# netneurolab/pypyls

Hardware: AMD Instinct MI355X
Metric: resamples/sec (perm+boot), behavioral_pls X(500x200000)/Y(500x50) fp64 (higher is better)
Workload: dtype f64

## Files before the change

### pypyls_amd/csrc/plsx_core.hip

```cpp
#include "plsx_internal.h"
#include "plsx_resample.h"
using namespace plsxi;

namespace plsxi {

const char* const kKernelClassNames[KC_COUNT] = {"k_xprod", "k_gram", "k_small", "k_urot", "k_nt_gemm",
                                                 "k_ucorr_partial", "k_simpls_dual", "k_build_A", "k_xprod_moments",
                                                 "k_sd_cv_score", "k_sd_coef", "k_coef_prod", "k_percentile", "k_contrast", "k_mb_rownorm"};

int plan_groups(plsx_ctx* c)
{
    const bool mb = c->method == PLSX_MULTIBLOCK;
    c->scaled = ((c->method == PLSX_BEHAVIORAL || mb) && !c->cov) ? 1 : 0;
    c->momrows = ((c->method == PLSX_BEHAVIORAL && (!c->cov || c->cv_mom)) || (mb && !c->cov)) ? 1 : 0;
    const int Jw = c->momrows ? c->J : 0;
    c->gps = 0;
    c->h_slice_row0.clear(); c->h_slice_rows.clear(); c->h_slice_cell0.clear(); c->h_slice_ncell.clear();
    auto fit = [&](int mt) {
        int b = 0;
        for (int n = 1; n <= 512; ++n) {
            int td = ceil_div(n * c->Tp, 16), tw = Jw ? ceil_div(n * Jw, 16) : 0;
            if (td + 2 * tw <= mt && tw * 16 <= 48) b = n; else break;
        }
        return b;
// ... 202 lines not shown
        if (waste < 0.03) break;
    }
    return best;
}

SmallArgs small_args(plsx_ctx* ctx, int mode)
{
    SmallArgs a;
    memset(&a, 0, sizeof(a));
    a.mode = mode; a.n = ctx->Tp; a.L = ctx->L; a.rotate = 1;
    a.G = ptr<double>(ctx->Gm); a.P = ptr<double>(ctx->Pm);
    a.V0 = ptr<double>(ctx->V0); a.d0 = ptr<double>(ctx->d0);
    a.Mfrag = ptr<double>(ctx->Mfrag); a.nks_t = ctx->nks_t; a.LT = ctx->LT;
    a.status = ptr<int>(ctx->status);
    return a;
}

bool plsc_single_pass(const plsx_ctx* ctx)
{
    return ctx->method != PLSX_REGRESSION && !ctx->scaled && use_dual(ctx) && ctx->gps == 0 && ctx->L == ctx->Tp &&
           ctx->Tp <= PLSX_JACOBI_TP && 2 * (size_t)ctx->L * PLSX_ACC_PITCH * 8 <= 72 * 1024 && !ctx->opt[OPT_TWO_PASS_BOOT];
}

int note_spectrum(plsx_ctx* ctx, const double* d_sv, hipStream_t st)
{
    std::vector<double> d(ctx->L);
    HIPCHK(hipMemcpyAsync(d.data(), d_sv, (size_t)ctx->L * 8, hipMemcpyDeviceToHost, st));
    HIPCHK(hipStreamSynchronize(st));
    double dmax = 0.0;
    for (double v : d) if (v > dmax) dmax = v;
    int graded = 0;
    for (double v : d) if (v > PLSX_RANK_RTOL * dmax && v < PLSX_REFINE_TAU * dmax) graded = 1;
    if (graded != ctx->graded) ctx->has_Kd = ctx->has_Kd && !graded;
    ctx->graded = graded && !ctx->opt[OPT_NO_REFINE];
    return 0;
}

int run_contrast_norms(plsx_ctx* ctx, int nres, double* out_sv, hipStream_t st)
{
    const int ntiles = ceil_div(ctx->B, 16);
    const int tpc = std::max(32, round_up(ceil_div(ntiles, 64), 4));
    const int nchunk = ceil_div(ntiles, tpc);
    const int LTl = ceil_div(ctx->nc, 16);
    if (int e = ensure(ctx, ctx->cpart, (size_t)nres * nchunk * ctx->L * 8)) return e;
    KTimer tm(ctx, KC_CONTRAST, st);
    for (int lt0 = 0; lt0 < LTl; lt0 += 4) {
        const int ltc = std::min(4, LTl - lt0);
        const size_t lds = (size_t)ctx->nks_t * ltc * 512;
        const bool vlds = lds <= 64 * 1024;
#define CN_ARGS ptr<double>(ctx->R), ctx->strideR, ctx->Bpad, ctx->nks_t, ptr<double>(ctx->Cfrag), ctx->LT, lt0, ctx->B, \
                tpc, ctx->L, ptr<double>(ctx->cpart)
#define CN_CASE(N) case N: \
            if (vlds) { HIPCHK(set_lds((k_contrast_norms<N, true>), lds)); \
                        hipLaunchKernelGGL((k_contrast_norms<N, true>), dim3(nchunk, nres), dim3(256), lds, st, CN_ARGS); } \
            else hipLaunchKernelGGL((k_contrast_norms<N, false>), dim3(nchunk, nres), dim3(256), 0, st, CN_ARGS); \
// ... 44 lines not shown
    if (!c) return PLSX_ERR_HIP;
    c->device = device;
    if (hipMalloc(&c->status.p, 4 * sizeof(int)) != hipSuccess || hipMemset(c->status.p, 0, 4 * sizeof(int)) != hipSuccess) {
        delete c;
        return PLSX_ERR_HIP;
    }
    c->status.bytes = 4 * sizeof(int);
    *out = c;
    return PLSX_OK;
} PLSX_CATCH(nullptr)

int plsx_ctx_destroy(plsx_ctx* ctx)
try {
    if (!ctx) return PLSX_OK;
    (void)hipSetDevice(ctx->device);
    (void)hipDeviceSynchronize();
    (void)plsx_comm_destroy(ctx);
    for (Buf* b : {&ctx->Xc, &ctx->xmean, &ctx->Y, &ctx->cell_of_row, &ctx->cell_start, &ctx->cell_len,
                   &ctx->out_row, &ctx->mom_idx, &ctx->mom_n, &ctx->Afrag, &ctx->R, &ctx->Gm, &ctx->Pm,
                   &ctx->part, &ctx->Mfrag, &ctx->U0T, &ctx->V0, &ctx->d0, &ctx->tmpW,
                   &ctx->Rfull, &ctx->Vp, &ctx->dp, &ctx->Mvd, &ctx->Cm, &ctx->srcx, &ctx->srcy, &ctx->part2,
                   &ctx->Kmat, &ctx->swork, &ctx->spct, &ctx->sc,
                   &ctx->momout, &ctx->R2, &ctx->cvc, &ctx->Qm, &ctx->Vs, &ctx->ds, &ctx->ybar, &ctx->pred,
                   &ctx->Xn, &ctx->out_row_f, &ctx->mom_idx_f, &ctx->Kd, &ctx->Ad, &ctx->Wd, &ctx->gws, &ctx->cellS, &ctx->rowc, &ctx->out_row_s, &ctx->okx, &ctx->oky, &ctx->psum, &ctx->psq, &ctx->row_slice, &ctx->row_local, &ctx->slice_cell0, &ctx->cell_momrow, &ctx->status, &ctx->ScT, &ctx->out_row_w, &ctx->Qs, &ctx->out_row_d, &ctx->mom_idx_d, &ctx->Afrag_m, &ctx->momn_m, &ctx->scale,
                   &ctx->Afrag_c, &ctx->rank_c, &ctx->rowtab_c, &ctx->m1_c, &ctx->m2_c, &ctx->out_row_c, &ctx->mom_idx_c, &ctx->mask_c,
                   &ctx->refV, &ctx->refLam, &ctx->refK0, &ctx->refPart, &ctx->refPartP, &ctx->refH, &ctx->flipws, &ctx->pflags,
                   &ctx->Cq, &ctx->Vsumq, &ctx->Vdq, &ctx->Cc, &ctx->Asumc, &ctx->Adc, &ctx->Qc, &ctx->cichunk, &ctx->cpA, &ctx->cppart, &ctx->colsd, &ctx->Zcv, &ctx->cvpsrc, &ctx->cvpfit, &ctx->shrsum, &ctx->shq, &ctx->shG, &ctx->shKG, &ctx->Vtq, &ctx->Afrag_q, &ctx->qpart, &ctx->ccon, &ctx->sFt, &ctx->Yrot,
                   &ctx->Cv, &ctx->Cfrag, &ctx->cpart, &ctx->mbpart})
        release(*b);
    for (auto& ev : ctx->events) { (void)hipEventDestroy(ev.e0); (void)hipEventDestroy(ev.e1); }
    delete ctx;
    return PLSX_OK;
} PLSX_CATCH(ctx)

const char* plsx_last_error(const plsx_ctx* ctx) { return ctx ? ctx->err.c_str() : "null context"; }

int plsx_sync(plsx_ctx* ctx)
try {
    if (!ctx) return PLSX_ERR_ARG;
    HIPCHK(hipSetDevice(ctx->device));
    HIPCHK(hipDeviceSynchronize());
    int stw[4] = {0, 0, 0, 0};
    HIPCHK(hipMemcpy(stw, ctx->status.p, 4 * sizeof(int), hipMemcpyDeviceToHost));
    if (stw[1] || stw[2]) {
        ctx->n_refined += stw[1];
        ctx->n_unrefined += stw[2];
        HIPCHK(hipMemset(static_cast<int*>(ctx->status.p) + 1, 0, 2 * sizeof(int)));
// ... 312 lines not shown
try {
    NEED_DATA();
    if (!d_W || !d_out || L < 1) return fail(ctx, PLSX_ERR_ARG, "plsx_project: bad arguments");
    hipStream_t st = static_cast<hipStream_t>(stream);
    HIPCHK(hipSetDevice(ctx->device));
    if (int e = ensure(ctx, ctx->tmpW, (size_t)L * ctx->Bpad * 8)) return e;
    HIPCHK(hipMemsetAsync(ctx->tmpW.p, 0, (size_t)L * ctx->Bpad * 8, st));
    hipLaunchKernelGGL(k_transpose, dim3(ceil_div(L, 32), ceil_div(ctx->B, 32)), dim3(32, 8), 0, st,
                       d_W, ctx->B, L, L, ptr<double>(ctx->tmpW), ctx->Bpad);
    LAUNCHCHK();
    return run_nt(ctx, ptr<double>(ctx->Xc), 0, ctx->Bpad, ctx->S, ptr<double>(ctx->tmpW), 0, ctx->Bpad, L,
                  nullptr, 0, 0, 0, ctx->B, 1, d_out, 0, L, nullptr, 0, 0, st);
} PLSX_CATCH(ctx)

int plsx_set_original(plsx_ctx* ctx, const double* d_xw, const double* d_sv, const double* d_yw,
                      void* stream)
try {
    NEED_DATA();
    if (!d_xw || !d_sv || !d_yw) return fail(ctx, PLSX_ERR_ARG, "plsx_set_original: null input");
    hipStream_t st = static_cast<hipStream_t>(stream);
    HIPCHK(hipSetDevice(ctx->device));
    HIPCHK(hipMemcpyAsync(ctx->V0.p, d_yw, (size_t)ctx->Tp * ctx->L * 8, hipMemcpyDeviceToDevice, st));
    HIPCHK(hipMemcpyAsync(ctx->d0.p, d_sv, (size_t)ctx->L * 8, hipMemcpyDeviceToDevice, st));
    if (int e = note_spectrum(ctx, d_sv, st)) return e;
    hipLaunchKernelGGL(k_transpose, dim3(ceil_div(ctx->L, 32), ceil_div(ctx->B, 32)), dim3(32, 8), 0, st,
                       d_xw, ctx->B, ctx->L, ctx->L, ptr<double>(ctx->U0T), ctx->Bpad);
    LAUNCHCHK();
    if (int e = run_nt(ctx, ptr<double>(ctx->Xc), 0, ctx->Bpad, ctx->S, ptr<double>(ctx->U0T), 0, ctx->Bpad,
                       ctx->L, nullptr, 0, 0, 0, ctx->B, 1, ptr<double>(ctx->Xc) + ctx->B, 0, ctx->Bpad,
                       nullptr, 0, 0, st))
        return e;
    {
        const int Sd = round_up(ctx->S, 8);
        if (int e = ensure(ctx, ctx->ScT, (size_t)ctx->L * Sd * 8, true)) return e;
        HIPCHK(hipMemsetAsync(ctx->ScT.p, 0, (size_t)ctx->L * Sd * 8, st));
        hipLaunchKernelGGL(k_transpose, dim3(ceil_div(ctx->L, 32), ceil_div(ctx->S, 32)), dim3(32, 8), 0, st,
                           ptr<double>(ctx->Xc) + ctx->B, ctx->S, ctx->L, ctx->Bpad, ptr<double>(ctx->ScT), Sd);
        LAUNCHCHK();
    }
    ctx->has_orig = true; ctx->quad_active = 0;
    return PLSX_OK;
} PLSX_CATCH(ctx)

}

namespace plsxi {

// ... 61 lines not shown
                               ptr<int>(ctx->cell_of_row), idx, lay, ptr<double>(ctx->Ad), (size_t)0, Sd,
                               -1);
        }
        LAUNCHCHK();
        if (int e = run_nt(ctx, ptr<double>(ctx->Ad), 0, Sd, m * Tp, ptr<double>(ctx->Kd), 0, Sd, S,
                           nullptr, 0, 0, 0, S, 1, ptr<double>(ctx->Wd), 0, Sd, nullptr, 0, 0, st))
            return e;
        if (int e = run_dual_gp(ctx, m, Sd, nullptr, 0, st)) return e;
        if (ctx->nc > 0) {
            KTimer tm(ctx, KC_CONTRAST, st);
            hipLaunchKernelGGL(k_contrast_quad, dim3(m), dim3(256), 0, st, ptr<double>(ctx->Gm), Tp, ptr<double>(ctx->Cv),
                               ctx->L, ctx->nc, d_out_sv + (size_t)off * ctx->L);
            LAUNCHCHK();
            continue;
        }
        SmallArgs a = small_args(ctx, SMALL_PERM);
        a.rotate = rotate ? 1 : 0;
        a.out_sv = d_out_sv + (size_t)off * ctx->L;
        if (int e = run_small(ctx, a, m, st)) return e;
    }
    return PLSX_OK;
}

int perm_batch_impl(plsx_ctx* ctx, const int32_t* d_perm_idx, const double* d_ystack, int n, int rotate,
                    double* d_out_sv, void* stream)
{
    hipStream_t st = static_cast<hipStream_t>(stream);
    HIPCHK(hipSetDevice(ctx->device));
    if (use_dual(ctx)) return perm_dual(ctx, d_perm_idx, d_ystack, n, rotate, d_out_sv, st);
    const int pg = ctx->fix ? ctx->npgf : ctx->npg;
    const int nb = balanced_batch(n, launch_groups(ctx, n, pg) * pg, pg);
    for (int off = 0; off < n; off += nb) {
        const int m = std::min(nb, n - off);
        const int* idx = d_perm_idx ? d_perm_idx + (size_t)off * ctx->S : nullptr;
        const bool perm_y = ctx->method == PLSX_BEHAVIORAL || ctx->method == PLSX_MULTIBLOCK;
        const int* xs = perm_y ? nullptr : idx;
        const int* ys = perm_y ? idx : nullptr;
        const double* yst = d_ystack ? d_ystack + (size_t)off * ctx->S * ctx->T : nullptr;
        if (ctx->fix) {
            if (int e = run_xprod_fixed(ctx, ys, m, st, yst)) return e;
        } else if (int e = run_xprod(ctx, xs, ys, m, st, false, yst)) return e;
        if (ctx->nc > 0) {
            if (int e = run_contrast_norms(ctx, m, d_out_sv + (size_t)off * ctx->L, st)) return e;
            continue;
        }
        if (int e = run_gram(ctx, m, false, st)) return e;
        SmallArgs a = small_args(ctx, SMALL_PERM);
        a.rotate = rotate ? 1 : 0;
        a.out_sv = d_out_sv + (size_t)off * ctx->L;
        if (int e = run_small(ctx, a, m, st, ptr<double>(ctx->R))) return e;
    }
    return PLSX_OK;
}

}

namespace plsxi {

int quad_accumulate(plsx_ctx* ctx, int m, hipStream_t st, const QuadSet* qs)
{
    const int S = ctx->S, L = qs ? qs->L : (ctx->method == PLSX_REGRESSION ? ctx->ncomp : ctx->L);
// ... 394 lines not shown
try {
    plsx_ctx* ctx = const_cast<plsx_ctx*>(cctx);
    if (!ctx || !out || cap < 1) return PLSX_ERR_ARG;
    double ms = 0.0;
    int launches = 0;
    for (auto& ev : ctx->events) {
        if (ev.cls != KC_XPROD) continue;
        float t = 0.f;
        if (hipEventSynchronize(ev.e1) == hipSuccess && hipEventElapsedTime(&t, ev.e0, ev.e1) == hipSuccess)
            ms += t;
        ++launches;
    }
    double crows = 0.0;
    if (ctx->last_compact_n > 0) {
        std::vector<int> cnt(ctx->last_compact_n);
        if (hipMemcpy(cnt.data(), ptr<int>(ctx->rowtab_c) + (size_t)ctx->last_compact_n * ctx->last_compact_ktot,
                      cnt.size() * sizeof(int), hipMemcpyDeviceToHost) == hipSuccess) {
            for (int c : cnt) crows += 4.0 * ((std::max(c, 1) + 3) / 4);
            crows /= (double)cnt.size() * ctx->S;
        }
    }
    const bool cmp = ctx->last_compact_n > 0;
    const auto uvar = [&](int nks) { return (double)(nks > 0 && ctx->urot_tail_l ? nks + 100 : nks); };
    double vals[22] = {ms, (double)launches, (double)(cmp ? 1 : (ctx->sepmom_used ? ctx->npg_d : ctx->npg)),
                       (double)(cmp ? ceil_div(ctx->Tp, 16) : (ctx->sepmom_used ? ctx->MTd : ctx->MT)),
                       (double)ctx->Gcap * ctx->npg, (double)ctx->timed_units, (double)use_dual(ctx), crows,
                       ctx->nt_flops, (double)ctx->quad_series, (double)ctx->quad_MT, (double)ctx->quad_gpl,
                       (double)ctx->urot_waves_l, (double)ctx->urot_splits_l, (double)ctx->urot_rps_l,
                       uvar(ctx->urot_nks_first), (double)ctx->gram_chunks_l, uvar(ctx->urot_nks_last),
                       (double)ctx->gram_kind_l, (double)ctx->split_blocks_l, (double)ctx->split_reader_l,
                       (double)(cmp && ctx->last_moment_rows ? 1 : 0)};
    int n = std::min(cap, 22);
    for (int i = 0; i < n; ++i) out[i] = vals[i];
    return n;
} PLSX_CATCH(const_cast<plsx_ctx*>(cctx))

int plsx_kernel_timing(const plsx_ctx* cctx, int kernel_class, double* ms_out, int* launches_out)
try {
    plsx_ctx* ctx = const_cast<plsx_ctx*>(cctx);
    if (!ctx || kernel_class < 0 || kernel_class >= KC_COUNT) return PLSX_ERR_ARG;
    double ms = 0.0;
    int launches = 0;
    for (auto& ev : ctx->events) {
        if (ev.cls != kernel_class) continue;
        float t = 0.f;
        if (hipEventSynchronize(ev.e1) == hipSuccess && hipEventElapsedTime(&t, ev.e0, ev.e1) == hipSuccess)
            ms += t;
        ++launches;
    }
    if (ms_out) *ms_out = ms;
    if (launches_out) *launches_out = launches;
    return PLSX_OK;
} PLSX_CATCH(const_cast<plsx_ctx*>(cctx))

const char* plsx_kernel_class_name(int kernel_class)
// ... 146 lines not shown
```

### pypyls_amd/csrc/plsx_internal.h

```cpp
#pragma once
#include "plsx_kernels.h"
#include <chrono>
#include "../../include/plsx.h"

#include <algorithm>
#include <cmath>
#include <cstdio>
#include <cstdlib>
#include <cstring>
#include <new>
#include <stdexcept>
#include <string>
#include <thread>
#include <vector>

struct Buf {
    void* p = nullptr;
    size_t bytes = 0;
};

enum {
    OPT_NO_REFINE = 0, OPT_MIN_BATCH, OPT_INBLOCK_MOMENTS, OPT_NO_COMPACT_BOOT, OPT_COMPACT_BOOT_ALWAYS,
    OPT_SEPMOM_ALWAYS, OPT_NO_GRAM4, OPT_UROT_GENERIC, OPT_UROT_NO_TAIL4, OPT_NO_FIXED_X, OPT_NO_DUAL_PERM,
    OPT_TWO_PASS_BOOT, OPT_SPLIT_INBLOCK, OPT_NO_SPLIT_FUSE, OPT_SPLIT_TWO_READERS, OPT_EXPECT_RESAMPLES,
    OPT_SIMPLS_JACOBI, OPT_PERCENTILE_SORT, OPT_QUAD_SUMS, OPT_SPLIT_READER8, OPT_SIMPLS_GLOBAL,
    OPT_CROSSCOV_SPARSE, OPT_NO_MOMENT_ROWS, OPT_COUNT
};
static const char* const kOptionNames[OPT_COUNT] = {
    "no_refine", "min_batch", "inblock_moments", "no_compact_boot", "compact_boot_always",
    "sepmom_always", "no_gram4", "urot_generic", "urot_no_tail4", "no_fixed_x", "no_dual_perm",
    "two_pass_boot", "split_inblock", "no_split_fuse", "split_two_readers", "expect_resamples",
    "simpls_jacobi", "percentile_sort", "quad_sums", "split_reader8", "simpls_global",
    "crosscov_sparse", "no_moment_rows"};

#ifndef PLSX_CKT
#define PLSX_CKT 3
#endif

struct plsx_ctx {
    int device = 0;
    std::string err;
    int opt[OPT_COUNT] = {};
    bool has_data = false, has_orig = false;
    int method = 0, S = 0, B = 0, T = 0, J = 0, n_groups = 0, n_cond = 1, mc = 0, cov = 0;
    int Tp = 0, Tpp = 0, L = 0, Kpad = 0, nks = 0, Bx = 0, Bpad = 0;
    int MT = 24, npg = 0, w0 = 0, sq0 = 0, nmom_pad = 0, scaled = 0, momrows = 0, Gcap = 0, Galloc = 0;
    int nks_t = 0, LT = 0, cv_mom = 0;
    int afrag_group0 = 0;
    int sepmom = 0, MTd = 0, npg_d = 0, sepmom_used = 0;
    size_t group_stride_d = 0;
    Buf out_row_d, mom_idx_d, Afrag_m, momn_m, scale;
    Buf Afrag_c, rank_c, rowtab_c, m1_c, m2_c, out_row_c, mom_idx_c, mask_c;
    int has_compact_maps = 0;
    size_t group_stride = 0;
    int gps = 0;
    Buf row_slice, row_local, slice_cell0, cell_momrow;
// ... 11 lines not shown
    Buf Kd, Ad, Wd;
    Buf Zcv;
    Buf cvpsrc, cvpfit;
    Buf shrsum, shq, shG, shKG;
    int has_shrsum = 0;
    Buf Qs;
    Buf ScT, out_row_w;
    int npg_w = 0;
    Buf gws;
    Buf status;
    Buf pflags;
    Buf flipws;
    Buf refV, refLam, refK0, refPart, refPartP, refH, Yrot;
    int graded = 0;
    long long n_refined = 0, n_unrefined = 0;
    Buf cellS, rowc, out_row_s;
    Buf ccon, sFt;
    int split_blocks_l = 0, split_reader_l = 0;
    int has_sFt = 0, split_raw = 0;
    int has_cellS = 0;
    int nc = 0;
    Buf Cv, Cfrag, cpart;
    Buf mbpart;
    int dual = 0, dual_ok = 0, has_Kd = 0;
    Buf okx, oky;
    Buf psum, psq;
    Buf Cq, Vsumq, Vdq, Vtq, Afrag_q, qpart;
    int quad_active = 0;
    long long quad_n = 0, series_total = 0;
    Buf Cc, Asumc, Adc, Qc;
    int coef_active = 0, coef_c = 0;
    long long coef_n = 0;
    double* keepA = nullptr;
    long long keep_cap = 0, keep_n = 0;
    Buf cichunk;
    double* vipG = nullptr;
    long long vip_cap = 0, vip_n = 0;
    int vip_c = 0;
    int cperm_active = 0, cperm_c = 0, cperm_std = 0;
    const double* cperm_obs = nullptr;
    int* cperm_count = nullptr;
    double* cperm_max = nullptr;
    long long cperm_cap = 0, cperm_n = 0;
    Buf cpA, cppart, colsd;
    bool has_okx = false, has_oky = false;
    int n_okx = 0;
// ... 133 lines not shown
    if (base + ints * 4 > 60 * 1024) { *cap = 0; return base; }
    *cap = (int)ints;
    return base + ints * 4;
}
inline size_t build_lds_mc(const plsx_ctx* ctx, int* cap)
{
    const size_t ints = (size_t)2 * ctx->S;
    if (ints * 4 > 60 * 1024) { *cap = 0; return 0; }
    *cap = (int)ints;
    return ints * 4;
}

int plan_groups(plsx_ctx* c);
int upload_rowmaps(plsx_ctx* ctx);
int plan_sepmom(plsx_ctx* ctx);
int ensure_scratch(plsx_ctx* ctx, int groups);
int launch_groups(plsx_ctx* ctx, long long units, int per_group);
int balanced_batch(int n, int cap, int per_group);
void probe_map_cost(plsx_ctx* ctx);
int chip_slots(const void* kernel);
int pick_parts(long long units, int slots, int lo, int hi);
SmallArgs small_args(plsx_ctx* ctx, int mode);
bool plsc_single_pass(const plsx_ctx* ctx);
int note_spectrum(plsx_ctx* ctx, const double* d_sv, hipStream_t st);
struct QuadSet { Buf* C; Buf* Vsum; const double* Vd; int L; };
int quad_accumulate(plsx_ctx* ctx, int m, hipStream_t st, const QuadSet* qs = nullptr);
bool quad_applicable(const plsx_ctx* ctx);
int run_contrast_norms(plsx_ctx* ctx, int nres, double* out_sv, hipStream_t st);
int run_contrast_fill(plsx_ctx* ctx, int nres, hipStream_t st);
int run_percentile(plsx_ctx* ctx, const double* d_data, long long nseries, int n, int i_lo, double g_lo, int i_hi,
                   double g_hi, double* d_lo, double* d_hi, hipStream_t st);
inline void coef_close(plsx_ctx* ctx)
{
    ctx->coef_active = 0; ctx->coef_n = 0;
    ctx->keepA = nullptr; ctx->keep_cap = 0; ctx->keep_n = 0;
}
inline void vip_close(plsx_ctx* ctx)
{
    ctx->vipG = nullptr; ctx->vip_cap = 0; ctx->vip_n = 0; ctx->vip_c = 0;
}
inline void cperm_close(plsx_ctx* ctx)
{
    ctx->cperm_active = 0; ctx->cperm_c = 0; ctx->cperm_std = 0;
    ctx->cperm_obs = nullptr; ctx->cperm_count = nullptr; ctx->cperm_max = nullptr;
    ctx->cperm_cap = 0; ctx->cperm_n = 0;
}
int launch_xprod(plsx_ctx* ctx, int groups, hipStream_t st);
int launch_xprod_acc(plsx_ctx* ctx, const double* Afrag, size_t gstride, int groups, int L, hipStream_t st);
int run_xprod_fixed(plsx_ctx* ctx, const int* ysrc, int nres, hipStream_t st, const double* ystack);
MomLayout moment_layout(const plsx_ctx* ctx, int npairs);
MomLayout moment2_layout(const plsx_ctx* ctx, int npairs);
int compact_boot_ksteps(int mt);
bool compact_moment_rows(const plsx_ctx* ctx);
int launch_moment_blocks_raw(plsx_ctx* ctx, const MomLayout& ml, SplitEpi se, hipStream_t st);
int ensure_compact_maps(plsx_ctx* ctx);
int run_mb_rownorm(plsx_ctx* ctx, int nres, hipStream_t st);
int run_xprod(plsx_ctx* ctx, const int* xsrc, const int* ysrc, int nres, hipStream_t st,
              bool prebuilt = false, const double* ystack = nullptr, long long ystride = -1, bool sparse_rows = false);
int launch_xprod_split(plsx_ctx* ctx, int groups, SplitEpi se, hipStream_t st);
int quad_finish(plsx_ctx* ctx, double* d_usum, double* d_usq, hipStream_t st, const QuadSet* qs = nullptr);
inline int quad_blocks(int tiles) { return tiles >= 8 ? ceil_div(tiles, 8) : 1; }
int launch_cboot(plsx_ctx* ctx, int nres, int nks_c, SplitEpi se, hipStream_t st);
int launch_csplit(plsx_ctx* ctx, int m, int nks_c, SplitEpi se, hipStream_t st, bool raw = false);
int run_nt(plsx_ctx* ctx, const double* A, long long strideA, int lda, int Ma,
           const double* B1, long long strideB1, int ldb1, int N1,
           const double* B2, long long strideB2, int ldb2, int N2, int K, int batch,
           double* C1, long long strideC1, int ldc1, double* C2, long long strideC2, int ldc2,
           hipStream_t st, bool sym = false, bool accumulate = false, bool one_chunk = false);
bool nt_sym_fits(int S);
int nt_strips(plsx_ctx* ctx, const double* A, int lda, int Ma, const double* Bm, int ldb, int N, int Kc,
              double* C, int ldc, hipStream_t st, bool one_chunk = false);
int form_gram_K(plsx_ctx* ctx, const double* X, int ldx, int S, int Kc, double* K, int ldk, hipStream_t st);
// ... 18 lines not shown
```

### pypyls_amd/csrc/plsx_k_contrast.h

```cpp
#pragma once
#include "plsx_common.h"
#include "plsx_k_small.h"


__device__ __forceinline__ size_t cfrag_tile_base(int lt, int nks_t, int LT, int& ltc)
{
    const int chunk = lt / PLSX_LT_CHUNK;
    ltc = min(PLSX_LT_CHUNK, LT - chunk * PLSX_LT_CHUNK);
    return mfrag_chunk_base(chunk, nks_t) + (size_t)(lt - chunk * PLSX_LT_CHUNK) * 64;
}

static __global__ void k_contrast_pack(const double* __restrict__ C, int n, int Lc, int L, int nks_t, int LT,
                                       double* __restrict__ dense, double* __restrict__ frag)
{
    const int idx = blockIdx.x * blockDim.x + threadIdx.x;
    if (idx < n * L) {
        const int t = idx / L, l = idx - t * L;
        dense[idx] = l < Lc ? C[(size_t)t * Lc + l] : 0.0;
    }
    if (idx < nks_t * LT * 64) {
        int lane, lt, ks;
        mfrag_decode(idx, nks_t, LT, ks, lt, lane);
        const int t = ks * 4 + (lane >> 4), l = lt * 16 + (lane & 15);
        frag[idx] = (t < n && l < Lc) ? C[(size_t)t * Lc + l] : 0.0;
// ... 79 lines not shown
        v += __shfl_xor(v, 32);
        if (lane < 16) red[wave][j][lane] = v;
    }
    __syncthreads();
    if (threadIdx.x < LTC * 16) {
        const int j = threadIdx.x >> 4, c = threadIdx.x & 15, l = (lt0 + j) * 16 + c;
        if (l < L)
            partial[((size_t)r * nchunk + chunk) * L + l] = ((red[0][j][c] + red[1][j][c]) + red[2][j][c]) + red[3][j][c];
    }
}

static __global__ void k_contrast_finish(const double* __restrict__ partial, int nchunk, int nres, int L, int Lc,
                                         double* __restrict__ out)
{
    const long long idx = (long long)blockIdx.x * blockDim.x + threadIdx.x;
    if (idx >= (long long)nres * L) return;
    const int r = (int)(idx / L), l = (int)(idx - (long long)r * L);
    double s = 0.0;
    if (l < Lc)
        for (int c = 0; c < nchunk; ++c) s += partial[((size_t)r * nchunk + c) * L + l];
    out[idx] = sqrt(s);
}

static __global__ void k_contrast_quad(const double* __restrict__ G, int n, const double* __restrict__ V, int L, int Lc,
                                       double* __restrict__ out)
{
    const double* Gr = G + (size_t)blockIdx.x * n * n;
    for (int l = threadIdx.x; l < L; l += blockDim.x) {
        double q = 0.0;
        if (l < Lc)
            for (int i = 0; i < n; ++i) {
                double t = 0.0;
                for (int j = 0; j < n; ++j) t += Gr[(size_t)i * n + j] * V[(size_t)j * L + l];
                q += V[(size_t)i * L + l] * t;
            }
        out[(size_t)blockIdx.x * L + l] = sqrt(fmax(q, 0.0));
    }
}

static __global__ void k_contrast_scale(double* __restrict__ Z, long long count, int L, const double* __restrict__ sv)
{
    const long long idx = (long long)blockIdx.x * blockDim.x + threadIdx.x;
    if (idx >= count) return;
    const double s = sv[idx % L];
    Z[idx] = s > 0.0 ? Z[idx] / s : 0.0;
}
// ... 1 lines not shown
```

### pypyls_amd/csrc/plsx_k_prep.h

```cpp
#pragma once
#include "plsx_common.h"


static __global__ void k_colmean(const double* __restrict__ X, int S, int B, double* __restrict__ mean)
{
    int b = blockIdx.x * blockDim.x + threadIdx.x;
    if (b >= B) return;
    double s = 0.0;
    for (int i = 0; i < S; ++i) s += X[(size_t)i * B + b];
    mean[b] = s / (double)S;
}

static __global__ void k_center_pad(const double* __restrict__ X, const double* __restrict__ mean,
                             int S, int B, double* __restrict__ Xc, int ldx)
{
    int b = blockIdx.x * blockDim.x + threadIdx.x;
    int i = blockIdx.y;
    if (b >= B || i >= S) return;
    Xc[(size_t)i * ldx + b] = X[(size_t)i * B + b] - mean[b];
}

static __global__ void k_cell_scale(const double* __restrict__ Xc, int ldx, int B, int J,
                             const int* __restrict__ cell_start, const int* __restrict__ cell_len,
                             double* __restrict__ Xn)
// ... 162 lines not shown
        const int mrow = pair % mom_pairs, mmt = mom_row0 >= 0 ? mom_pairs / 16 : mom_pairs / 8;
        for (int pl = tid; pl < len; pl += blockDim.x) {
            int p = start + pl;
            int xi = xs ? xs[p] : p;
            if (xi < 0) continue;
            if (mom_row0 >= 0)
                put_weight(A + afrag_off(mom_row0 + j, rank[(size_t)r * S + xi], lay.MT), Am + afrag_off(mrow, xi, mmt), pl);
            else
                put_weight(Am + afrag_off(mrow, xi, mmt), Am + afrag_off(mom_pairs + mrow, xi, mmt), pl);
        }
        if (tid == 0) mom_n[pair] = (double)cnt;
    } else if (scaled) {
        for (int pl = tid; pl < len; pl += blockDim.x) {
            int p = start + pl;
            int xi = xs ? xs[p] : p;
            if (xi < 0) continue;
            int mrow = rr * lay.J + j;
            put_weight(A + afrag_off(lay.w0 * 16 + mrow, xi, lay.MT), A + afrag_off(lay.sq0 * 16 + mrow, xi, lay.MT), pl);
        }
        if (tid == 0) mom_n[(size_t)g * nmom_pad + rr * lay.J + j] = (double)cnt;
    }
}

static __global__ void k_build_A_mc(int S, int J, int n_cond, int mean_centering,
                             const int* __restrict__ cell_of_pos,
                             const int* __restrict__ xsrc, GroupLayout lay,
                             double* __restrict__ Afrag, size_t group_stride, int dense_ld = 0, int chain_cap = 0)
{
    extern __shared__ int sm_mc[];
    __shared__ int cnt[PLSX_MAX_CELLS];
    const int r = blockIdx.x;
    const int g = r / lay.n, rr = r % lay.n;
    const int* xs = xsrc ? xsrc + (size_t)r * S : nullptr;
    const int tid = threadIdx.x;
    for (int j = tid; j < J; j += blockDim.x) cnt[j] = 0;
    __syncthreads();
    for (int p = tid; p < S; p += blockDim.x)
        if ((xs ? xs[p] : p) >= 0) atomicAdd(&cnt[cell_of_pos[p]], 1);
    __syncthreads();
    const int n_groups = J / n_cond;
    int ntot = 0;
    for (int j = 0; j < J; ++j) ntot += cnt[j];
    double* A = Afrag + (size_t)g * group_stride;
    int* nxt = sm_mc;
    int* nfirst = sm_mc + S;
    const bool unique = !xs || chain_cap < 0;
// ... 276 lines not shown
```

### pypyls_amd/csrc/plsx_k_xprod.h

```cpp
#pragma once
#include <type_traits>
#include <utility>

template <class F, int... I>
__device__ __forceinline__ void xprod_static_for(F&& f, std::integer_sequence<int, I...>)
{
    (f(std::integral_constant<int, I>()), ...);
}
#include "plsx_common.h"
#include "plsx_k_prep.h"

#define PLSX_RSRC_FLAGS 0x00020000
template <int NT, int PASSES, bool EVEN, int STAGE>
__device__ __forceinline__ void stage_copy_buf(const double* src, double* dst, int tid, int wave)
{
    __amdgpu_buffer_rsrc_t rs = __builtin_amdgcn_make_buffer_rsrc((void*)src, (short)0, 0x7fffffff,
                                                                   PLSX_RSRC_FLAGS);
    const int voff = tid * 16;
#pragma unroll
    for (int p = 0; p < PASSES; ++p) {
        if (EVEN || p * NT + wave * 64 < STAGE / 2) {
            __builtin_amdgcn_raw_ptr_buffer_load_lds(
                rs, (__attribute__((address_space(3))) void*)(dst + (size_t)(p * NT + wave * 64) * 2),
                16, voff, p * NT * 16, 0, 0);
        }
    }
}

__device__ __forceinline__ double load_x_buf(const double* rowbase, int voff)
{
    __amdgpu_buffer_rsrc_t rs = __builtin_amdgcn_make_buffer_rsrc((void*)rowbase, (short)0, 0x7fffffff,
                                                                   PLSX_RSRC_FLAGS);
    return __builtin_bit_cast(double, __builtin_amdgcn_raw_buffer_load_b64(rs, voff, 0, 0));
}

#define PLSX_ACC_PITCH 80
template <int MT, int NW, int KT, int NSQ, int EPI = 0>
__global__ __launch_bounds__(NW * 64, 2)
void k_xprod(const double* __restrict__ Afrag, size_t group_stride,
             const double* __restrict__ X, int ldx, int nks,
             double* __restrict__ R, int ldr, int rows_per_group,
             const int* __restrict__ out_row, const int* __restrict__ mom_idx,
             const double* __restrict__ mom_n, int nmom_pad,
             int n_groups, int ncolblk, double* __restrict__ mom_out, SplitEpi se, int ntab)
{
    extern __shared__ __attribute__((aligned(16))) double smem[];
    constexpr int NT = NW * 64;
    constexpr int STAGE = KT * MT * 64;
    constexpr int STAGE_LDS = ((STAGE + 127) / 128) * 128;
    constexpr int PASSES = (STAGE + NT * 2 - 1) / (NT * 2);
    constexpr bool EVEN = (STAGE % (NT * 2)) == 0;
    const int tid = threadIdx.x;
    const int lane = tid & 63, wave = tid >> 6;
    const int sweep = blockIdx.x / (8 * ncolblk);
    const int within = blockIdx.x - sweep * (8 * ncolblk);
    int grp = sweep * 8 + (within & 7);
// ... 65 lines not shown
            const double bsq = (NSQ > 0) ? b * b : 0.0;
#pragma unroll
            for (int m = 0; m < NA; ++m)
                acc[m] = mfma_f64(sA[(s * MT + m) * 64], (m < MT - NSQ) ? b : bsq, acc[m]);
        }
#pragma unroll
        for (int s = 0; s < KT; ++s) xb[s] = xn[s];
        __syncthreads();
    };
    int kt_first = 0;
    if constexpr (EPI == 7) {
        xprod_static_for([&](auto mm) {
#pragma unroll
            for (int j = 0; j < 4 / KT; ++j) {
                const int kt = (4 / KT) * decltype(mm)::value + j;
                if (kt < nkt) pass(kt, std::integral_constant<int, decltype(mm)::value + 1>());
            }
        }, std::make_integer_sequence<int, MT>());
        kt_first = min(nkt, 4 * MT / KT);
    }
    for (int kt = kt_first; kt < nkt; ++kt) pass(kt, std::integral_constant<int, MT>());

    constexpr int W0 = (EPI == 9) ? 0 : MT - 2 * NSQ, SQ0 = MT - NSQ, NMOM = NSQ * 16;
    if constexpr (EPI == 9) {
        static_assert(MT == NSQ, "EPI 9 runs every tile against X^2");
#pragma unroll
        for (int j = 0; j < MT; ++j)
#pragma unroll
            for (int i = 0; i < 4; ++i) {
                const int pair = grp * (MT * 16) + j * 16 + kq + 4 * i;
                if (pair >= se.npairs || col >= ldr) continue;
                se.scale[(size_t)pair * ldr + col] = acc[j][i];
            }
        return;
    }
    if constexpr (EPI == 6) {
        static_assert(MT == 2 * NSQ, "EPI 6 is a moment-only instantiation");
#pragma unroll
        for (int j = 0; j < NSQ; ++j)
#pragma unroll
            for (int i = 0; i < 4; ++i) {
                const int pair = grp * (NSQ * 16) + j * 16 + kq + 4 * i;
                if (pair >= se.npairs || col >= ldr) continue;
                se.scale[(size_t)pair * ldr + col] = acc[j][i];
                se.scale2[(size_t)pair * ldr + col] = acc[NSQ + j][i];
            }
// ... 590 lines not shown
```

### pypyls_amd/csrc/plsx_xprod.hip

```cpp
#include "plsx_internal.h"

using namespace plsxi;

namespace plsxi {

template <int MT, int NW, int KT, int NSQ>
int launch_xprod_t(plsx_ctx* ctx, int groups, hipStream_t st)
{
    const size_t stage = (size_t)2 * (((size_t)KT * MT * 64 + 127) / 128) * 128 * 8;
    const size_t epi = (size_t)NW * 2 * NSQ * 16 * 16 * 8 + (size_t)2 * MT * 16 * 4;
    const size_t lds = std::max(stage, epi);
    HIPCHK(set_lds(k_xprod<MT, NW, KT, NSQ>, lds));
    const int ncolblk = ctx->Bpad / (NW * 16);
    dim3 grid(ncolblk * round_up(groups, 8)), block(NW * 64);
    KTimer tm(ctx, KC_XPROD, st);
    hipLaunchKernelGGL((k_xprod<MT, NW, KT, NSQ>), grid, block, lds, st,
                       ptr<double>(ctx->Afrag) + (size_t)ctx->afrag_group0 * ctx->group_stride, ctx->group_stride,
                       ptr<double>(ctx->Xc), ctx->Bpad,
                       ctx->nks, ptr<double>(ctx->R), ctx->Bpad, ctx->npg * ctx->Tpp,
                       ptr<int>(ctx->out_row), ptr<int>(ctx->mom_idx), ptr<double>(ctx->mom_n),
                       std::max(ctx->nmom_pad, 0), groups, ncolblk, ctx->mom_out_arg,
                       SplitEpi{nullptr, nullptr, nullptr, nullptr, nullptr, 0, 0}, std::max(ctx->gps, 1));
    LAUNCHCHK();
    return 0;
// ... 98 lines not shown
{
    const int groups = ceil_div(nres, ctx->npgf);
    if (int e = ensure_scratch(ctx, groups)) return e;
    if (ctx->timing) ctx->timed_units += nres;
    ctx->last_compact_n = 0;
    HIPCHK(hipMemsetAsync(ctx->Afrag.p, 0, (size_t)groups * ctx->group_stride_f * 8, st));
    GroupLayout lay;
    lay.n = ctx->npgf; lay.Tp = ctx->Tp; lay.J = ctx->J; lay.T = ctx->T; lay.MT = ctx->MTf;
    lay.w0 = ctx->MTf; lay.sq0 = ctx->MTf; lay.Tpp = ctx->Tpp;
    {
        dim3 grid(nres, ctx->J), block(256);
        const size_t lds = (size_t)2 * ctx->T * 8;
        hipLaunchKernelGGL(k_build_A_behav, grid, block, lds, st, ystack ? ystack : ptr<double>(ctx->Y),
                           ystack ? (long long)ctx->S * ctx->T : 0LL, ctx->T, ctx->S,
                           ptr<int>(ctx->cell_start), ptr<int>(ctx->cell_len), (const int*)nullptr, ysrc, lay,
                           0, 0, ptr<double>(ctx->Afrag), ctx->group_stride_f, ptr<double>(ctx->mom_n), 16);
        LAUNCHCHK();
    }
    switch (stage_ksteps(ctx->nks)) {
        case 3: return launch_xprod_fixed_t<3>(ctx, groups, st);
        case 2: return launch_xprod_fixed_t<2>(ctx, groups, st);
        default: return launch_xprod_fixed_t<1>(ctx, groups, st);
    }
}

template <int MT>
int launch_xprod_data(plsx_ctx* ctx, int groups, SplitEpi se, hipStream_t st)
{
    constexpr int NW = 4, KT = 1;
    const size_t stage = (size_t)2 * (((size_t)KT * MT * 64 + 127) / 128) * 128 * 8;
    const size_t epi = (size_t)se.npairs * NW * 16 * 8 + (size_t)2 * MT * 16 * 4;
    const size_t lds = std::max(stage, epi);
    HIPCHK(set_lds(k_xprod<MT, NW, KT, 0, 3>, lds));
    const int ncolblk = ctx->Bpad / (NW * 16);
    KTimer tm(ctx, KC_XPROD, st);
    hipLaunchKernelGGL((k_xprod<MT, NW, KT, 0, 3>), dim3(ncolblk * round_up(groups, 8)), dim3(NW * 64), lds, st,
                       ptr<double>(ctx->Afrag), ctx->group_stride_d, ptr<double>(ctx->Xc), ctx->Bpad, ctx->nks,
                       ptr<double>(ctx->R), ctx->Bpad, ctx->npg_d * ctx->Tpp, ptr<int>(ctx->out_row_d),
                       ptr<int>(ctx->mom_idx_d), (const double*)nullptr, 0, groups, ncolblk, (double*)nullptr, se, 1);
    LAUNCHCHK();
    return 0;
}

int run_xprod_sepmom(plsx_ctx* ctx, const int* xsrc, const int* ysrc, int nres, hipStream_t st,
                     const double* ystack, long long ystride)
{
// ... 349 lines not shown
```

### pypyls_amd/engine.py

```python
import ctypes
import threading
import os

import numpy as np

from . import _build

_LIB = None

PLSX_BEHAVIORAL = 0
PLSX_MEANCENTERED = 1
PLSX_REGRESSION = 2
PLSX_FLAG_COVARIANCE = 1


class PlsxError(RuntimeError):
    pass


def _load():
    global _LIB
    if _LIB is not None:
        return _LIB
    import torch
# ... 826 lines not shown
        self._check(self.lib.plsx_set_timing(self.ctx, 1 if enable else 0))

    def kernel_timing(self):
        out = {}
        k = 0
        while True:
            name = self.lib.plsx_kernel_class_name(k)
            if not name:
                break
            ms, n = ctypes.c_double(), ctypes.c_int()
            self._check(self.lib.plsx_kernel_timing(self.ctx, k, ctypes.byref(ms), ctypes.byref(n)))
            if n.value:
                out[name.decode()] = (ms.value, n.value)
            k += 1
        return out

    def set_perm_path(self, dual):
        rc = self.lib.plsx_set_perm_path(self.ctx, -1 if dual is None else (1 if dual else 0))
        if rc < 0:
            self._check(rc)
        return bool(rc)

    def last_timing(self):
        buf = (ctypes.c_double * 22)()
        n = self.lib.plsx_last_timing(self.ctx, buf, 22)
        keys = ['xprod_ms', 'xprod_launches', 'resamples_per_group', 'm_tiles', 'superbatch',
                'xprod_resamples', 'dual_perm', 'compact_row_fraction', 'nt_flops', 'quad_series', 'quad_m_tiles',
                'quad_blocks_per_lv', 'urot_waves', 'urot_splits', 'urot_res_per_split', 'urot_variant',
                'gram_chunks', 'urot_variant_last', 'gram_kernel', 'split_blocks', 'split_reader',
                'moment_rows']
        return {k: buf[i] for i, k in enumerate(keys[:max(n, 0)])}


_DEFAULT = {}
_DEFAULT_LOCK = threading.Lock()


def default_engine(device=None, replica=0):
    torch = _torch()
    if device is None:
        device = torch.cuda.current_device() if torch.cuda.is_available() else 0
    key = (int(device), int(replica))
    with _DEFAULT_LOCK:
        eng = _DEFAULT.get(key)
        if eng is None or not getattr(eng, 'ctx', None):
            if not _DEFAULT:
                import atexit
                atexit.register(release_default_engine)
            eng = _DEFAULT[key] = Engine(device=key[0])
    return eng


IDLE_RELEASE_S = 300.0
# ... 47 lines not shown
```

Before: 5754.

## Project permuted Y onto original saliences and compute permutation singular values as row norms

Adds a projected permutation path. With fixed X, rotation on, no contrasts and full rank, it folds the original V0 saliences into the A matrix (k_build_A_proj) so that the cross-product directly yields projected rows. Their squared norms are reduced inside a new xprod epilogue (EPI 10, DPP row reductions plus per-block partials) and finished by a small kernel. This avoids writing the full R matrix and running the small SVD/rotation stage per permutation. The cost is an extra partials buffer and a numerically different rotation-based estimate that holds only when the original spectrum is fully live.

New measurement: 6149 (median of 6 runs). 1.07x the previous value.

```diff
diff --git a/pypyls_amd/csrc/plsx_core.hip b/pypyls_amd/csrc/plsx_core.hip
--- a/pypyls_amd/csrc/plsx_core.hip
+++ b/pypyls_amd/csrc/plsx_core.hip
@@ -248,7 +248,7 @@
            ctx->Tp <= PLSX_JACOBI_TP && 2 * (size_t)ctx->L * PLSX_ACC_PITCH * 8 <= 72 * 1024 && !ctx->opt[OPT_TWO_PASS_BOOT];
 }
 
-int note_spectrum(plsx_ctx* ctx, const double* d_sv, hipStream_t st)
+int note_spectrum(plsx_ctx* ctx, const double* d_sv, hipStream_t st, int* all_live)
 {
     std::vector<double> d(ctx->L);
     HIPCHK(hipMemcpyAsync(d.data(), d_sv, (size_t)ctx->L * 8, hipMemcpyDeviceToHost, st));
@@ -257,6 +257,7 @@
     for (double v : d) if (v > dmax) dmax = v;
     int graded = 0;
     for (double v : d) if (v > PLSX_RANK_RTOL * dmax && v < PLSX_REFINE_TAU * dmax) graded = 1;
+    if (all_live) *all_live = (ctx->L > 0 && d[ctx->L - 1] > PLSX_RANK_RTOL * d[0]) ? 1 : 0;
     if (graded != ctx->graded) ctx->has_Kd = ctx->has_Kd && !graded;
     ctx->graded = graded && !ctx->opt[OPT_NO_REFINE];
     return 0;
@@ -347,7 +348,7 @@
                    &ctx->Rfull, &ctx->Vp, &ctx->dp, &ctx->Mvd, &ctx->Cm, &ctx->srcx, &ctx->srcy, &ctx->part2,
                    &ctx->Kmat, &ctx->swork, &ctx->spct, &ctx->sc,
                    &ctx->momout, &ctx->R2, &ctx->cvc, &ctx->Qm, &ctx->Vs, &ctx->ds, &ctx->ybar, &ctx->pred,
-                   &ctx->Xn, &ctx->out_row_f, &ctx->mom_idx_f, &ctx->Kd, &ctx->Ad, &ctx->Wd, &ctx->gws, &ctx->cellS, &ctx->rowc, &ctx->out_row_s, &ctx->okx, &ctx->oky, &ctx->psum, &ctx->psq, &ctx->row_slice, &ctx->row_local, &ctx->slice_cell0, &ctx->cell_momrow, &ctx->status, &ctx->ScT, &ctx->out_row_w, &ctx->Qs, &ctx->out_row_d, &ctx->mom_idx_d, &ctx->Afrag_m, &ctx->momn_m, &ctx->scale,
+                   &ctx->Xn, &ctx->ppart, &ctx->out_row_f, &ctx->mom_idx_f, &ctx->Kd, &ctx->Ad, &ctx->Wd, &ctx->gws, &ctx->cellS, &ctx->rowc, &ctx->out_row_s, &ctx->okx, &ctx->oky, &ctx->psum, &ctx->psq, &ctx->row_slice, &ctx->row_local, &ctx->slice_cell0, &ctx->cell_momrow, &ctx->status, &ctx->ScT, &ctx->out_row_w, &ctx->Qs, &ctx->out_row_d, &ctx->mom_idx_d, &ctx->Afrag_m, &ctx->momn_m, &ctx->scale,
                    &ctx->Afrag_c, &ctx->rank_c, &ctx->rowtab_c, &ctx->m1_c, &ctx->m2_c, &ctx->out_row_c, &ctx->mom_idx_c, &ctx->mask_c,
                    &ctx->refV, &ctx->refLam, &ctx->refK0, &ctx->refPart, &ctx->refPartP, &ctx->refH, &ctx->flipws, &ctx->pflags,
                    &ctx->Cq, &ctx->Vsumq, &ctx->Vdq, &ctx->Cc, &ctx->Asumc, &ctx->Adc, &ctx->Qc, &ctx->cichunk, &ctx->cpA, &ctx->cppart, &ctx->colsd, &ctx->Zcv, &ctx->cvpsrc, &ctx->cvpfit, &ctx->shrsum, &ctx->shq, &ctx->shG, &ctx->shKG, &ctx->Vtq, &ctx->Afrag_q, &ctx->qpart, &ctx->ccon, &ctx->sFt, &ctx->Yrot,
@@ -706,7 +707,8 @@
     HIPCHK(hipSetDevice(ctx->device));
     HIPCHK(hipMemcpyAsync(ctx->V0.p, d_yw, (size_t)ctx->Tp * ctx->L * 8, hipMemcpyDeviceToDevice, st));
     HIPCHK(hipMemcpyAsync(ctx->d0.p, d_sv, (size_t)ctx->L * 8, hipMemcpyDeviceToDevice, st));
-    if (int e = note_spectrum(ctx, d_sv, st)) return e;
+    ctx->orig_all_live = 0;
+    if (int e = note_spectrum(ctx, d_sv, st, &ctx->orig_all_live)) return e;
     hipLaunchKernelGGL(k_transpose, dim3(ceil_div(ctx->L, 32), ceil_div(ctx->B, 32)), dim3(32, 8), 0, st,
                        d_xw, ctx->B, ctx->L, ctx->L, ptr<double>(ctx->U0T), ctx->Bpad);
     LAUNCHCHK();
@@ -814,12 +816,21 @@
     return PLSX_OK;
 }
 
+bool perm_projected(const plsx_ctx* ctx, int rotate)
+{
+    return ctx->fix && rotate && ctx->nc == 0 && ctx->L == ctx->Tp && ctx->has_orig && ctx->orig_all_live &&
+           !ctx->opt[OPT_NO_PERM_PROJECT];
+}
+
 int perm_batch_impl(plsx_ctx* ctx, const int32_t* d_perm_idx, const double* d_ystack, int n, int rotate,
                     double* d_out_sv, void* stream)
 {
     hipStream_t st = static_cast<hipStream_t>(stream);
     HIPCHK(hipSetDevice(ctx->device));
+    ctx->last_perm_projected = 0;
     if (use_dual(ctx)) return perm_dual(ctx, d_perm_idx, d_ystack, n, rotate, d_out_sv, st);
+    const bool projected = perm_projected(ctx, rotate);
+    ctx->last_perm_projected = projected ? 1 : 0;
     const int pg = ctx->fix ? ctx->npgf : ctx->npg;
     const int nb = balanced_batch(n, launch_groups(ctx, n, pg) * pg, pg);
     for (int off = 0; off < n; off += nb) {
@@ -829,6 +840,10 @@
         const int* xs = perm_y ? nullptr : idx;
         const int* ys = perm_y ? idx : nullptr;
         const double* yst = d_ystack ? d_ystack + (size_t)off * ctx->S * ctx->T : nullptr;
+        if (projected) {
+            if (int e = run_xprod_fixed_norms(ctx, ys, m, st, yst, d_out_sv + (size_t)off * ctx->L)) return e;
+            continue;
+        }
         if (ctx->fix) {
             if (int e = run_xprod_fixed(ctx, ys, m, st, yst)) return e;
         } else if (int e = run_xprod(ctx, xs, ys, m, st, false, yst)) return e;
@@ -1269,15 +1284,15 @@
     }
     const bool cmp = ctx->last_compact_n > 0;
     const auto uvar = [&](int nks) { return (double)(nks > 0 && ctx->urot_tail_l ? nks + 100 : nks); };
-    double vals[22] = {ms, (double)launches, (double)(cmp ? 1 : (ctx->sepmom_used ? ctx->npg_d : ctx->npg)),
+    double vals[23] = {ms, (double)launches, (double)(cmp ? 1 : (ctx->sepmom_used ? ctx->npg_d : ctx->npg)),
                        (double)(cmp ? ceil_div(ctx->Tp, 16) : (ctx->sepmom_used ? ctx->MTd : ctx->MT)),
                        (double)ctx->Gcap * ctx->npg, (double)ctx->timed_units, (double)use_dual(ctx), crows,
                        ctx->nt_flops, (double)ctx->quad_series, (double)ctx->quad_MT, (double)ctx->quad_gpl,
                        (double)ctx->urot_waves_l, (double)ctx->urot_splits_l, (double)ctx->urot_rps_l,
                        uvar(ctx->urot_nks_first), (double)ctx->gram_chunks_l, uvar(ctx->urot_nks_last),
                        (double)ctx->gram_kind_l, (double)ctx->split_blocks_l, (double)ctx->split_reader_l,
-                       (double)(cmp && ctx->last_moment_rows ? 1 : 0)};
-    int n = std::min(cap, 22);
+                       (double)(cmp && ctx->last_moment_rows ? 1 : 0), (double)ctx->last_perm_projected};
+    int n = std::min(cap, 23);
     for (int i = 0; i < n; ++i) out[i] = vals[i];
     return n;
 } PLSX_CATCH(const_cast<plsx_ctx*>(cctx))
diff --git a/pypyls_amd/csrc/plsx_internal.h b/pypyls_amd/csrc/plsx_internal.h
--- a/pypyls_amd/csrc/plsx_internal.h
+++ b/pypyls_amd/csrc/plsx_internal.h
@@ -24,14 +24,14 @@
     OPT_SEPMOM_ALWAYS, OPT_NO_GRAM4, OPT_UROT_GENERIC, OPT_UROT_NO_TAIL4, OPT_NO_FIXED_X, OPT_NO_DUAL_PERM,
     OPT_TWO_PASS_BOOT, OPT_SPLIT_INBLOCK, OPT_NO_SPLIT_FUSE, OPT_SPLIT_TWO_READERS, OPT_EXPECT_RESAMPLES,
     OPT_SIMPLS_JACOBI, OPT_PERCENTILE_SORT, OPT_QUAD_SUMS, OPT_SPLIT_READER8, OPT_SIMPLS_GLOBAL,
-    OPT_CROSSCOV_SPARSE, OPT_NO_MOMENT_ROWS, OPT_COUNT
+    OPT_CROSSCOV_SPARSE, OPT_NO_MOMENT_ROWS, OPT_NO_PERM_PROJECT, OPT_COUNT
 };
 static const char* const kOptionNames[OPT_COUNT] = {
     "no_refine", "min_batch", "inblock_moments", "no_compact_boot", "compact_boot_always",
     "sepmom_always", "no_gram4", "urot_generic", "urot_no_tail4", "no_fixed_x", "no_dual_perm",
     "two_pass_boot", "split_inblock", "no_split_fuse", "split_two_readers", "expect_resamples",
     "simpls_jacobi", "percentile_sort", "quad_sums", "split_reader8", "simpls_global",
-    "crosscov_sparse", "no_moment_rows"};
+    "crosscov_sparse", "no_moment_rows", "no_perm_project"};
 
 #ifndef PLSX_CKT
 #define PLSX_CKT 3
@@ -89,6 +89,9 @@
     int nc = 0;
     Buf Cv, Cfrag, cpart;
     Buf mbpart;
+    Buf ppart;
+    int orig_all_live = 0;
+    int last_perm_projected = 0;
     int dual = 0, dual_ok = 0, has_Kd = 0;
     Buf okx, oky;
     Buf psum, psq;
@@ -268,7 +271,7 @@
 int pick_parts(long long units, int slots, int lo, int hi);
 SmallArgs small_args(plsx_ctx* ctx, int mode);
 bool plsc_single_pass(const plsx_ctx* ctx);
-int note_spectrum(plsx_ctx* ctx, const double* d_sv, hipStream_t st);
+int note_spectrum(plsx_ctx* ctx, const double* d_sv, hipStream_t st, int* all_live = nullptr);
 struct QuadSet { Buf* C; Buf* Vsum; const double* Vd; int L; };
 int quad_accumulate(plsx_ctx* ctx, int m, hipStream_t st, const QuadSet* qs = nullptr);
 bool quad_applicable(const plsx_ctx* ctx);
@@ -294,6 +297,7 @@
 int launch_xprod(plsx_ctx* ctx, int groups, hipStream_t st);
 int launch_xprod_acc(plsx_ctx* ctx, const double* Afrag, size_t gstride, int groups, int L, hipStream_t st);
 int run_xprod_fixed(plsx_ctx* ctx, const int* ysrc, int nres, hipStream_t st, const double* ystack);
+int run_xprod_fixed_norms(plsx_ctx* ctx, const int* ysrc, int nres, hipStream_t st, const double* ystack, double* out_sv);
 MomLayout moment_layout(const plsx_ctx* ctx, int npairs);
 MomLayout moment2_layout(const plsx_ctx* ctx, int npairs);
 int compact_boot_ksteps(int mt);
diff --git a/pypyls_amd/csrc/plsx_k_contrast.h b/pypyls_amd/csrc/plsx_k_contrast.h
--- a/pypyls_amd/csrc/plsx_k_contrast.h
+++ b/pypyls_amd/csrc/plsx_k_contrast.h
@@ -125,6 +125,27 @@
     out[idx] = sqrt(s);
 }
 
+static __global__ void k_rownorm_finish(const double* __restrict__ part, int ncolblk, int groups, int rows, int n, int Tp,
+                                        int nres, double* __restrict__ out)
+{
+    const long long idx = (long long)blockIdx.x * blockDim.x + threadIdx.x;
+    if (idx >= (long long)nres * Tp) return;
+    const int r = (int)(idx / Tp), l = (int)(idx - (long long)r * Tp);
+    const double* p = part + (size_t)(r / n) * rows + (r % n) * Tp + l;
+    const size_t step = (size_t)groups * rows;
+    double s = 0.0;
+    int c = 0;
+    for (; c + 8 <= ncolblk; c += 8) {
+        double v[8];
+#pragma unroll
+        for (int u = 0; u < 8; ++u) v[u] = p[(size_t)(c + u) * step];
+#pragma unroll
+        for (int u = 0; u < 8; ++u) s += v[u];
+    }
+    for (; c < ncolblk; ++c) s += p[(size_t)c * step];
+    out[idx] = sqrt(s);
+}
+
 static __global__ void k_contrast_quad(const double* __restrict__ G, int n, const double* __restrict__ V, int L, int Lc,
                                        double* __restrict__ out)
 {
diff --git a/pypyls_amd/csrc/plsx_k_prep.h b/pypyls_amd/csrc/plsx_k_prep.h
--- a/pypyls_amd/csrc/plsx_k_prep.h
+++ b/pypyls_amd/csrc/plsx_k_prep.h
@@ -208,6 +208,49 @@
     }
 }
 
+static __global__ __launch_bounds__(256)
+void k_build_A_proj(const double* __restrict__ Y0, long long y_stride, int T, int S,
+                    const int* __restrict__ cell_start, const int* __restrict__ cell_len,
+                    const int* __restrict__ ysrc, const double* __restrict__ V0, int L,
+                    int n, int Tp, int MT, double* __restrict__ Afrag, size_t group_stride)
+{
+    extern __shared__ double sm_b[];
+    const int r = blockIdx.x, j = blockIdx.y;
+    const int g = r / n, rr = r % n;
+    const double* Y = Y0 + (size_t)r * y_stride;
+    const int start = cell_start[j], len = cell_len[j];
+    const int* ys = ysrc ? ysrc + (size_t)r * S : nullptr;
+    double* mean = sm_b;
+    double* rstd = sm_b + T;
+    const int tid = threadIdx.x;
+    for (int t = tid; t < T; t += blockDim.x) {
+        double s = 0.0;
+        for (int p = start; p < start + len; ++p) s += Y[(size_t)(ys ? ys[p] : p) * T + t];
+        const double m = s / (double)len;
+        double q = 0.0;
+        for (int p = start; p < start + len; ++p) {
+            const double d = Y[(size_t)(ys ? ys[p] : p) * T + t] - m;
+            q += d * d;
+        }
+        mean[t] = m;
+        rstd[t] = 1.0 / sqrt(q / (double)(len - 1));
+    }
+    __syncthreads();
+    double* A = Afrag + (size_t)g * group_stride;
+    const double inv_nm1 = 1.0 / (double)(len - 1);
+    const double* Vj = V0 + (size_t)j * T * L;
+    const int total = len * L;
+    for (int idx = tid; idx < total; idx += blockDim.x) {
+        const int pl = idx / L, l = idx - pl * L;
+        const int p = start + pl;
+        const double* y = Y + (size_t)(ys ? ys[p] : p) * T;
+        double v = 0.0;
+        for (int t = 0; t < T; ++t)
+            v = __builtin_fma((y[t] - mean[t]) * rstd[t] * inv_nm1, Vj[(size_t)t * L + l], v);
+        A[afrag_off(rr * Tp + l, p, MT)] = v;
+    }
+}
+
 static __global__ void k_build_A_mc(int S, int J, int n_cond, int mean_centering,
                              const int* __restrict__ cell_of_pos,
                              const int* __restrict__ xsrc, GroupLayout lay,
diff --git a/pypyls_amd/csrc/plsx_k_xprod.h b/pypyls_amd/csrc/plsx_k_xprod.h
--- a/pypyls_amd/csrc/plsx_k_xprod.h
+++ b/pypyls_amd/csrc/plsx_k_xprod.h
@@ -32,6 +32,15 @@
     __amdgpu_buffer_rsrc_t rs = __builtin_amdgcn_make_buffer_rsrc((void*)rowbase, (short)0, 0x7fffffff,
                                                                    PLSX_RSRC_FLAGS);
     return __builtin_bit_cast(double, __builtin_amdgcn_raw_buffer_load_b64(rs, voff, 0, 0));
+}
+
+template <int CTRL>
+__device__ __forceinline__ double dpp_row_f64(double v)
+{
+    const int vl = __double2loint(v), vh = __double2hiint(v);
+    const int lo = __builtin_amdgcn_update_dpp(vl, vl, CTRL, 0xf, 0xf, false);
+    const int hi = __builtin_amdgcn_update_dpp(vh, vh, CTRL, 0xf, 0xf, false);
+    return __hiloint2double(hi, lo);
 }
 
 #define PLSX_ACC_PITCH 80
@@ -143,6 +152,27 @@
     for (int kt = kt_first; kt < nkt; ++kt) pass(kt, std::integral_constant<int, MT>());
 
     constexpr int W0 = (EPI == 9) ? 0 : MT - 2 * NSQ, SQ0 = MT - NSQ, NMOM = NSQ * 16;
+    if constexpr (EPI == 10) {
+        static_assert(NSQ == 0 && NW == 4, "EPI 10 is the fixed-X block");
+        double* sP = smem;
+#pragma unroll
+        for (int m = 0; m < MT; ++m)
+#pragma unroll
+            for (int i = 0; i < 4; ++i) {
+                double q = acc[m][i] * acc[m][i];
+                q += dpp_row_f64<0x128>(q);
+                q += dpp_row_f64<0x124>(q);
+                q += dpp_row_f64<0x4e>(q);
+                q += dpp_row_f64<0xb1>(q);
+                if ((lane & 15) == 0) sP[wave * (MT * 16) + m * 16 + kq + 4 * i] = q;
+            }
+        __syncthreads();
+        const int rows = se.accB;
+        double* pp = se.acc_sum + ((size_t)colblk * n_groups + grp) * rows;
+        for (int row = tid; row < rows; row += NT)
+            pp[row] = ((sP[row] + sP[MT * 16 + row]) + sP[2 * MT * 16 + row]) + sP[3 * MT * 16 + row];
+        return;
+    }
     if constexpr (EPI == 9) {
         static_assert(MT == NSQ, "EPI 9 runs every tile against X^2");
 #pragma unroll
diff --git a/pypyls_amd/csrc/plsx_xprod.hip b/pypyls_amd/csrc/plsx_xprod.hip
--- a/pypyls_amd/csrc/plsx_xprod.hip
+++ b/pypyls_amd/csrc/plsx_xprod.hip
@@ -144,6 +144,60 @@
         case 2: return launch_xprod_fixed_t<2>(ctx, groups, st);
         default: return launch_xprod_fixed_t<1>(ctx, groups, st);
     }
+}
+
+template <int KT>
+int launch_xprod_fixed_norms_t(plsx_ctx* ctx, int groups, SplitEpi se, hipStream_t st)
+{
+    constexpr int MT = 25, NW = 4;
+    const size_t stage = (size_t)2 * (((size_t)KT * MT * 64 + 127) / 128) * 128 * 8;
+    const size_t lds = std::max(stage, (size_t)NW * MT * 16 * 8);
+    HIPCHK(set_lds(k_xprod<MT, NW, KT, 0, 10>, lds));
+    const int ncolblk = ctx->Bpad / (NW * 16);
+    dim3 grid(ncolblk * round_up(groups, 8)), block(NW * 64);
+    KTimer tm(ctx, KC_XPROD, st);
+    hipLaunchKernelGGL((k_xprod<MT, NW, KT, 0, 10>), grid, block, lds, st,
+                       ptr<double>(ctx->Afrag), ctx->group_stride_f, ptr<double>(ctx->Xn), ctx->Bpad,
+                       ctx->nks, (double*)nullptr, ctx->Bpad, ctx->npgf * ctx->Tpp,
+                       (const int*)nullptr, (const int*)nullptr, (const double*)nullptr, 0,
+                       groups, ncolblk, (double*)nullptr, se, 1);
+    LAUNCHCHK();
+    return 0;
+}
+
+int run_xprod_fixed_norms(plsx_ctx* ctx, const int* ysrc, int nres, hipStream_t st, const double* ystack, double* out_sv)
+{
+    const int groups = ceil_div(nres, ctx->npgf), rows = ctx->npgf * ctx->Tp;
+    const int ncolblk = ctx->Bpad / 64;
+    if (int e = ensure(ctx, ctx->Afrag, (size_t)groups * ctx->group_stride_f * 8 + 4096)) return e;
+    if (int e = ensure(ctx, ctx->ppart, (size_t)ncolblk * groups * rows * 8)) return e;
+    if (ctx->timing) ctx->timed_units += nres;
+    ctx->last_compact_n = 0;
+    HIPCHK(hipMemsetAsync(ctx->Afrag.p, 0, (size_t)groups * ctx->group_stride_f * 8, st));
+    {
+        KTimer tm(ctx, KC_BUILD, st);
+        hipLaunchKernelGGL(k_build_A_proj, dim3(nres, ctx->J), dim3(256), (size_t)2 * ctx->T * 8, st,
+                           ystack ? ystack : ptr<double>(ctx->Y), ystack ? (long long)ctx->S * ctx->T : 0LL, ctx->T, ctx->S,
+                           ptr<int>(ctx->cell_start), ptr<int>(ctx->cell_len), ysrc, ptr<double>(ctx->V0), ctx->L,
+                           ctx->npgf, ctx->Tp, ctx->MTf, ptr<double>(ctx->Afrag), ctx->group_stride_f);
+        LAUNCHCHK();
+    }
+    SplitEpi se;
+    memset(&se, 0, sizeof(se));
+    se.acc_sum = ptr<double>(ctx->ppart); se.accB = rows;
+    int e;
+    switch (stage_ksteps(ctx->nks)) {
+        case 3: e = launch_xprod_fixed_norms_t<3>(ctx, groups, se, st); break;
+        case 2: e = launch_xprod_fixed_norms_t<2>(ctx, groups, se, st); break;
+        default: e = launch_xprod_fixed_norms_t<1>(ctx, groups, se, st); break;
+    }
+    if (e) return e;
+    KTimer tm(ctx, KC_SMALL, st);
+    const long long count = (long long)nres * ctx->Tp;
+    hipLaunchKernelGGL(k_rownorm_finish, dim3((unsigned)((count + 255) / 256)), dim3(256), 0, st, ptr<double>(ctx->ppart),
+                       ncolblk, groups, rows, ctx->npgf, ctx->Tp, nres, out_sv);
+    LAUNCHCHK();
+    return 0;
 }
 
 template <int MT>
diff --git a/pypyls_amd/engine.py b/pypyls_amd/engine.py
--- a/pypyls_amd/engine.py
+++ b/pypyls_amd/engine.py
@@ -872,13 +872,13 @@
         return bool(rc)
 
     def last_timing(self):
-        buf = (ctypes.c_double * 22)()
-        n = self.lib.plsx_last_timing(self.ctx, buf, 22)
+        buf = (ctypes.c_double * 23)()
+        n = self.lib.plsx_last_timing(self.ctx, buf, 23)
         keys = ['xprod_ms', 'xprod_launches', 'resamples_per_group', 'm_tiles', 'superbatch',
                 'xprod_resamples', 'dual_perm', 'compact_row_fraction', 'nt_flops', 'quad_series', 'quad_m_tiles',
                 'quad_blocks_per_lv', 'urot_waves', 'urot_splits', 'urot_res_per_split', 'urot_variant',
                 'gram_chunks', 'urot_variant_last', 'gram_kernel', 'split_blocks', 'split_reader',
-                'moment_rows']
+                'moment_rows', 'perm_projected']
         return {k: buf[i] for i, k in enumerate(keys[:max(n, 0)])}
 
 
```
